# Snoworday/instance-segmentation-attention

Hardware: AMD Instinct MI355X
Metric: images/sec @256x256 bs=16 per GPU (higher is better)
Workload: dtype bf16; 1 GPU; train.py step fwd+bwd+update 256x256 bs=16/GPU (bf16); global_batch=16, parallelism=dp1, launch=hipGraph replay

## Files before the change

instance-segmentation-attention_amd/csrc/dwconv.hip:

```cpp
#include "common.hpp"
#include <type_traits>

namespace {

__device__ __forceinline__ void lds_barrier() {
    __builtin_amdgcn_fence(__ATOMIC_RELEASE, "workgroup", "local");
    __builtin_amdgcn_s_barrier();
    __builtin_amdgcn_fence(__ATOMIC_ACQUIRE, "workgroup", "local");
}

constexpr int TH = 8, TW = 32, CB = 32, PS = 36;
constexpr int HALO = (TH + 2) * (TW + 2);

struct Dw2Params {
    const void* x; const void* w; const float* bias; void* y; const void* dy;
    int n, h, w_, c, ldx, ldy, ldd, wld;
    ProDev pro;
    float* stats; int accumulate;
    int tiles_x, tiles_y; long ntiles;
    float* ws; int csrc;
    int G;
    FinDev fin;
};

// ... 18 lines not shown
    const int c0 = c_base + cg * 8;
    const bool cok = c0 < p.c;
    constexpr int NIT = (HALO * 4 + 255) / 256;
    float v[NIT][8];
    bool ok[NIT];
#pragma unroll
    for (int it = 0; it < NIT; ++it) {
        const int pix = (threadIdx.x + it * 256) >> 2;
        const int rr = pix / (TW + 2), cc = pix - rr * (TW + 2);
        const int gy = ty * TH + rr - 1, gx = tx * TW + cc - 1;
        ok[it] = pix < HALO && cok && gy >= 0 && gy < p.h && gx >= 0 && gx < p.w_;
        if (ok[it]) load8<T>(xin + (((long)b * p.h + gy) * p.w_ + gx) * p.ldx + c0, v[it]);
    }
#pragma unroll
    for (int it = 0; it < NIT; ++it) {
        const int pix = (threadIdx.x + it * 256) >> 2;
        if (pix >= HALO) continue;
        f32x4 a, bb;
#pragma unroll
        for (int j = 0; j < 8; ++j) {
            float z = 0.f;
            if (ok[it]) {
                z = v[it][j];
                if constexpr (HAS_PRO) {
                    z = act_t<ACT>(fmaf(z, r.sc[j], r.sh[j]), p.pro.act);
                    if (p.pro.bscale) z *= r.bs[j];
                }
            }
            if (j < 4) a[j] = z; else bb[j - 4] = z;
        }
        *reinterpret_cast<f32x4*>(tile + pix * PS + cg * 8) = a;
        *reinterpret_cast<f32x4*>(tile + pix * PS + cg * 8 + 4) = bb;
    }
}

typedef float f32x2 __attribute__((ext_vector_type(2)));
__device__ __forceinline__ void fma8(const float (&x)[8], const float (&w)[8], float (&acc)[8]) {
#ifdef ISA_DW_SCALAR_FMA
#pragma unroll
    for (int j = 0; j < 8; ++j) acc[j] = __builtin_fmaf(x[j], w[j], acc[j]);
#else
#pragma unroll
    for (int j = 0; j < 8; j += 2) {
        const f32x2 r = __builtin_elementwise_fma(f32x2{x[j], x[j + 1]}, f32x2{w[j], w[j + 1]}, f32x2{acc[j], acc[j + 1]});
        acc[j] = r[0]; acc[j + 1] = r[1];
    }
#endif
}

__device__ __forceinline__ void ld8(const float* p, float (&v)[8]) {
    const f32x4 a = *reinterpret_cast<const f32x4*>(p), b = *reinterpret_cast<const f32x4*>(p + 4);
#pragma unroll
    for (int j = 0; j < 4; ++j) { v[j] = a[j]; v[4 + j] = b[j]; }
}

struct TileRange { long t0, end, step; };
__device__ __forceinline__ TileRange tile_range(long ntiles, int bx, int nbx) {
    if ((nbx & 7) == 0 && ntiles >= 64) {
        const int xcd = bx & 7, j = bx >> 3;
        const long chunk = (ntiles + 7) / 8;
        const long end = min(ntiles, (xcd + 1) * chunk);
        return TileRange{xcd * chunk + j, end, (long)(nbx >> 3)};
    }
    return TileRange{(long)bx, ntiles, (long)nbx};
}

struct TileIter {
    long t, end, step;
    int tx, ty, b, sx, sy, sb, ntx, nty;
    __device__ __forceinline__ void init(const TileRange& r, int tiles_x, int tiles_y) {
        t = r.t0; end = r.end; step = r.step; ntx = tiles_x; nty = tiles_y;
        long q = t / tiles_x; tx = (int)(t - q * tiles_x); b = (int)(q / tiles_y); ty = (int)(q - (long)b * tiles_y);
        long qs = step / tiles_x; sx = (int)(step - qs * tiles_x); sb = (int)(qs / tiles_y); sy = (int)(qs - (long)sb * tiles_y);
    }
    __device__ __forceinline__ bool valid() const { return t < end; }
    __device__ __forceinline__ void next() {
        t += step;
        tx += sx; const int c = tx >= ntx ? 1 : 0; tx -= c * ntx;
        ty += sy + c; const int c2 = ty >= nty ? 1 : 0; ty -= c2 * nty;
        b += sb + c2;
    }
};

template <typename T, bool HAS_PRO, int ACT, bool DB>
__global__ __launch_bounds__(DB ? 768 : 256) __attribute__((amdgpu_waves_per_eu(2, 3))) void dw2_fwd_kernel(Dw2Params p) {
    constexpr int NTHR = DB ? 768 : 256;
    constexpr int LTHR = DB ? 512 : 256;
    constexpr int NBUF = DB ? 2 : 1;
    extern __shared__ __attribute__((aligned(16))) float sm[];
    float* tile_base = sm;
    float* wts = sm + NBUF * HALO * PS;
    float* red = wts + 9 * CB;
    float* fin_tab = red + 2 * CB;
    const int tid = threadIdx.x;
    const bool loader = DB && tid >= 256;
    const int ltid = loader ? tid - 256 : tid;
    const int c_base = blockIdx.y * CB;
    const GroupSel gs = group_sel(p.G);
    if (gs.g) {
        const long img = (long)gs.g * p.n, pix = img * p.h * p.w_;
        p.x = reinterpret_cast<const T*>(p.x) + pix * p.ldx;
        p.y = reinterpret_cast<T*>(p.y) + pix * p.ldy;
        p.pro.scale = goff(p.pro.scale, (long)gs.g * p.c); p.pro.shift = goff(p.pro.shift, (long)gs.g * p.c);
        p.pro.bscale = goff(p.pro.bscale, img * p.c);
        p.stats = goff(p.stats, (long)gs.g * ISA_STAT_R * 2 * p.c);
    }
    const T* wp = reinterpret_cast<const T*>(p.w);
    for (int i = tid; i < 9 * CB; i += NTHR) {
        const int tp = i / CB, cc = i - tp * CB;
        wts[i] = (c_base + cc < p.c) ? st<T>::ld(wp + (long)tp * p.wld + c_base + cc) : 0.f;
    }
    if (tid < 2 * CB) red[tid] = 0.f;
    const int cg = ltid & 3, g = ltid >> 2, row = g >> 3, x0 = (g & 7) * 4;
    const int c0 = c_base + cg * 8;
    const bool cok = c0 < p.c;
    const T* xin = reinterpret_cast<const T*>(p.x);
    constexpr int NIT = (HALO * 4 + LTHR - 1) / LTHR;

    const bool fin = HAS_PRO && bn_fin_inline<NTHR>(p.fin, p.c, p.G, gs.g, fin_tab, CB, tid, c_base, CB,
                                                    blockIdx.x == gridDim.x - 1 && blockIdx.z == 0);
    float sc[8], sh[8];
#pragma unroll
    for (int j = 0; j < 8; ++j) {
        const int c = min(c0 + j, p.c - 1);
        sc[j] = fin ? fin_tab[c - c_base] : ((HAS_PRO && p.pro.scale) ? p.pro.scale[c] : 1.f);
        sh[j] = fin ? fin_tab[CB + c - c_base] : ((HAS_PRO && p.pro.shift) ? p.pro.shift[c] : 0.f);
    }
    int hrc[NIT], hoff[NIT];
    bool hok[NIT];
#pragma unroll
    for (int it = 0; it < NIT; ++it) {
        const int pix = (ltid + it * LTHR) >> 2;
        const int rr = pix / (TW + 2), cc = pix - rr * (TW + 2);
        hrc[it] = (rr << 16) | cc;
        hoff[it] = (rr * p.w_ + cc) * p.ldx + (cok ? c0 : c_base);
        hok[it] = pix < HALO && cok;
    }
    const int ooff = (row * p.w_ + x0) * p.ldy + c0;

    auto stage = [&](int b, int ty, int tx, float* tile) {
        float bs[8];
        if (HAS_PRO && p.pro.bscale) {
#pragma unroll
            for (int j = 0; j < 8; ++j) bs[j] = p.pro.bscale[(long)b * p.c + min(c0 + j, p.c - 1)];
        }
        const T* base = xin + (((long)b * p.h + ty * TH - 1) * p.w_ + tx * TW - 1) * p.ldx;
        const int rlo = 1 - ty * TH, rhi = p.h + 1 - ty * TH, clo = 1 - tx * TW, chi = p.w_ + 1 - tx * TW;
        const bool interior = rlo <= 0 && rhi >= TH + 2 && clo <= 0 && chi >= TW + 2;
        raw8<T> v[NIT]; bool ok[NIT];
        if (interior) {
#pragma unroll
            for (int it = 0; it < NIT; ++it) { ok[it] = hok[it]; if (ok[it]) v[it].load(base + hoff[it]); }
        } else {
#pragma unroll
            for (int it = 0; it < NIT; ++it) {
                const int rr = hrc[it] >> 16, cc = hrc[it] & 0xffff;
                ok[it] = hok[it] && rr >= rlo && rr < rhi && cc >= clo && cc < chi;
                if (ok[it]) v[it].load(base + hoff[it]);
            }
        }
        const bool has_bs = HAS_PRO && p.pro.bscale;
#pragma unroll
        for (int it = 0; it < NIT; ++it) {
            const int pix = (ltid + it * LTHR) >> 2;
            if (pix >= HALO) continue;
            float o[8];
#pragma unroll
            for (int j = 0; j < 8; ++j) o[j] = 0.f;
            if (ok[it]) {
#pragma unroll
                for (int j = 0; j < 8; ++j) {
                    float z = v[it].get(j);
                    if constexpr (HAS_PRO) z = act_t<ACT>(fmaf(z, sc[j], sh[j]), p.pro.act);
                    o[j] = z;
                }
                if (has_bs) {
#pragma unroll
                    for (int j = 0; j < 8; ++j) o[j] *= bs[j];
                }
            }
            store8<float>(tile + pix * PS + cg * 8, o);
        }
    };

    auto compute = [&](int b, int ty, int tx, const float* tile, float (&s1)[8], float (&s2)[8]) {
        T* ybase = reinterpret_cast<T*>(p.y) + (((long)b * p.h + ty * TH) * p.w_ + tx * TW) * p.ldy;
        const bool rowok = ty * TH + row < p.h && cok;
        const int xlim = p.w_ - tx * TW;
        raw8<T> oc[4];
        if (p.accumulate && rowok) {
#pragma unroll
            for (int o = 0; o < 4; ++o)
                if (x0 + o < xlim) oc[o].load(ybase + ooff + o * p.ldy);
        }
        float acc[4][8];
        if (p.bias) {
#pragma unroll
            for (int o = 0; o < 4; ++o)
#pragma unroll
                for (int j = 0; j < 8; ++j) acc[o][j] = (c0 + j < p.c) ? p.bias[c0 + j] : 0.f;
        } else {
#pragma unroll
            for (int o = 0; o < 4; ++o)
#pragma unroll
                for (int j = 0; j < 8; ++j) acc[o][j] = 0.f;
        }
#pragma unroll 1
        for (int dy = 0; dy < 3; ++dy) {
            float wr[3][8], in[6][8];
#pragma unroll
            for (int k = 0; k < 3; ++k) ld8(wts + (dy * 3 + k) * CB + cg * 8, wr[k]);
#pragma unroll
            for (int k = 0; k < 6; ++k) ld8(tile + ((row + dy) * (TW + 2) + x0 + k) * PS + cg * 8, in[k]);
#pragma unroll
            for (int o = 0; o < 4; ++o)
#pragma unroll
                for (int k = 0; k < 3; ++k)
                    fma8(in[o + k], wr[k], acc[o]);
        }
        if (rowok) {
#pragma unroll
            for (int o = 0; o < 4; ++o) {
                if (x0 + o >= xlim) continue;
                T* dst = ybase + ooff + o * p.ldy;
#pragma unroll
                for (int j = 0; j < 8; ++j) { s1[j] += acc[o][j]; s2[j] += acc[o][j] * acc[o][j]; }
                if (p.accumulate) {
#pragma unroll
                    for (int j = 0; j < 8; ++j) acc[o][j] += oc[o].get(j);
                }
                store8<T>(dst, acc[o]);
            }
        }
    };

    __syncthreads();
    if (loader) {
        TileIter ti; ti.init(tile_range(p.ntiles, gs.bx, gs.nbx), p.tiles_x, p.tiles_y);
        int buf = 0;
        if (ti.valid()) stage(ti.b, ti.ty, ti.tx, tile_base);
        __syncthreads();
        while (ti.valid()) {
            ti.next();
            if (ti.valid()) stage(ti.b, ti.ty, ti.tx, tile_base + (buf ^ 1) * HALO * PS);
            lds_barrier();
            buf ^= 1;
        }
    } else {
        float s1[8] = {0, 0, 0, 0, 0, 0, 0, 0}, s2[8] = {0, 0, 0, 0, 0, 0, 0, 0};
        if constexpr (DB) {
            TileIter ti; ti.init(tile_range(p.ntiles, gs.bx, gs.nbx), p.tiles_x, p.tiles_y);
            int buf = 0;
            __syncthreads();
            for (; ti.valid(); ti.next()) {
                compute(ti.b, ti.ty, ti.tx, tile_base + buf * HALO * PS, s1, s2);
                lds_barrier();
                buf ^= 1;
            }
        } else {
            TileIter ti; ti.init(TileRange{(long)gs.bx, p.ntiles, (long)gs.nbx}, p.tiles_x, p.tiles_y);
            for (; ti.valid(); ti.next()) {
                stage(ti.b, ti.ty, ti.tx, tile_base);
                __syncthreads();
                compute(ti.b, ti.ty, ti.tx, tile_base, s1, s2);
                __syncthreads();
            }
        }
        if (p.stats) {
#pragma unroll
            for (int j = 0; j < 8; ++j) {
                s1[j] = row_fold<4>(s1[j]); s2[j] = row_fold<4>(s2[j]);
            }
            if ((tid & 15) < 4) {
#pragma unroll
                for (int j = 0; j < 8; ++j) { atomicAdd(&red[cg * 8 + j], s1[j]); atomicAdd(&red[CB + cg * 8 + j], s2[j]); }
            }
        }
    }
    __syncthreads();
    if (p.stats && tid < 2 * CB) {
        const int cc = tid & (CB - 1), which = tid / CB;
        if (c_base + cc < p.c && red[tid] != 0.f) {
            float* rep = p.stats + ((blockIdx.x + blockIdx.y) & (ISA_STAT_R - 1)) * 2 * p.c;
            atomicAdd(rep + which * p.c + c_base + cc, red[tid]);
        }
    }
}

template <typename T, bool HAS_PRO, int ACT>
__global__ __launch_bounds__(256) __attribute__((amdgpu_waves_per_eu(2, 2))) void dw2_wgrad_kernel(Dw2Params p) {
    extern __shared__ __attribute__((aligned(16))) float sm[];
    float* tile = sm;
    float* red = sm + HALO * PS;
    const int tid = threadIdx.x;
    const int c_base = blockIdx.y * CB;
    const int cg = tid & 3, g = tid >> 2, row = g >> 3, x0 = (g & 7) * 4;
    const int c0 = c_base + cg * 8;
    const GroupSel gs = group_sel(p.G);
    if (gs.g) {
        const long img = (long)gs.g * p.n, pix = img * p.h * p.w_;
        p.x = reinterpret_cast<const T*>(p.x) + pix * p.ldx;
        p.dy = reinterpret_cast<const T*>(p.dy) + pix * p.ldd;
        p.pro.scale = goff(p.pro.scale, (long)gs.g * p.c); p.pro.shift = goff(p.pro.shift, (long)gs.g * p.c);
        p.pro.bscale = goff(p.pro.bscale, img * p.c);
    }
    const T* din = reinterpret_cast<const T*>(p.dy);
    float acc[9][8], db[8];
#pragma unroll
    for (int tp = 0; tp < 9; ++tp)
#pragma unroll
        for (int j = 0; j < 8; ++j) acc[tp][j] = 0.f;
#pragma unroll
    for (int j = 0; j < 8; ++j) db[j] = 0.f;
    for (long t = gs.bx; t < p.ntiles; t += gs.nbx) {
        const int tx = (int)(t % p.tiles_x); const long q = t / p.tiles_x;
        const int ty = (int)(q % p.tiles_y); const int b = (int)(q / p.tiles_y);
        ProRegs pr;
        load_pro<HAS_PRO>(p, pr, c0, b);
        __syncthreads();
        stage_tile<T, HAS_PRO, ACT>(p, pr, tile, b, ty, tx, c_base);
        float d[4][8];
        const int oy = ty * TH + row;
#pragma unroll
        for (int o = 0; o < 4; ++o) {
            const int ox = tx * TW + x0 + o;
#pragma unroll
            for (int j = 0; j < 8; ++j) d[o][j] = 0.f;
            if (oy < p.h && ox < p.w_ && c0 < p.c) load8<T>(din + (((long)b * p.h + oy) * p.w_ + ox) * p.ldd + c0, d[o]);
        }
        __syncthreads();
#pragma unroll
        for (int o = 0; o < 4; ++o)
#pragma unroll
            for (int j = 0; j < 8; ++j) db[j] += d[o][j];
#pragma unroll
        for (int dy = 0; dy < 3; ++dy) {
            float in[6][8];
#pragma unroll
            for (int k = 0; k < 6; ++k) ld8(tile + ((row + dy) * (TW + 2) + x0 + k) * PS + cg * 8, in[k]);
#pragma unroll
            for (int o = 0; o < 4; ++o)
#pragma unroll
                for (int k = 0; k < 3; ++k)
                    fma8(in[o + k], d[o], acc[dy * 3 + k]);
            __builtin_amdgcn_sched_barrier(0);
        }
    }
    __syncthreads();
    for (int i = tid; i < 10 * CB; i += 256) red[i] = 0.f;
    __syncthreads();
#pragma unroll
    for (int tp = 0; tp < 10; ++tp) {
#pragma unroll
        for (int j = 0; j < 8; ++j) {
            float v = tp < 9 ? acc[tp < 9 ? tp : 0][j] : db[j];
            v = row_fold<4>(v);
            if ((tid & 15) < 4) atomicAdd(&red[tp * CB + cg * 8 + j], v);
        }
    }
    __syncthreads();
    float* slab = p.ws + ((long)blockIdx.x * gridDim.y + blockIdx.y) * 10 * CB;
    for (int i = tid; i < 10 * CB; i += 256) slab[i] = red[i];
}

constexpr int DW2_RSPLIT = 16;
__global__ __launch_bounds__(256) void dw2_wgrad_reduce_kernel(const float* ws, int nblk, int ncb, int C, int csrc, float* dw, float* dbias) {
    const int cb = blockIdx.x, split = blockIdx.y;
    const int per = (nblk + DW2_RSPLIT - 1) / DW2_RSPLIT;
    const int b0 = split * per, b1 = min(nblk, b0 + per);
    if (b0 >= b1) return;
    for (int i = threadIdx.x; i < 10 * CB; i += 256) {
        float s = 0.f;
#pragma unroll 8
        for (int b = b0; b < b1; ++b) s += ws[((long)b * ncb + cb) * 10 * CB + i];
        const int tp = i / CB, c = cb * CB + (i - tp * CB);
        if (c >= csrc || c >= C) continue;
        if (tp < 9) atomicAdd(dw + c * 9 + tp, s);
        else if (dbias) atomicAdd(dbias + c, s);
    }
}

template <typename T, bool HAS_PRO, int ACT>
int launch_fwd2_inst(Dw2Params& p, dim3 grid, hipStream_t s) {
    constexpr bool DB = sizeof(T) == 2;
    constexpr size_t lds = ((size_t)(DB ? 2 : 1) * HALO * PS + 9 * CB + 2 * CB + 2 * CB) * 4;
    static bool configured = false;
    if (!configured) {
        if (hipFuncSetAttribute(reinterpret_cast<const void*>(&dw2_fwd_kernel<T, HAS_PRO, ACT, DB>),
                                hipFuncAttributeMaxDynamicSharedMemorySize, (int)lds) != hipSuccess) return ISA_ELAUNCH;
        configured = true;
    }
    hipLaunchKernelGGL((dw2_fwd_kernel<T, HAS_PRO, ACT, DB>), grid, dim3(DB ? 768 : 256), lds, s, p);
    return launch_status();
}

template <typename T>
int launch_fwd2(Dw2Params& p, bool has_pro, hipStream_t s) {
    p.tiles_x = (p.w_ + TW - 1) / TW; p.tiles_y = (p.h + TH - 1) / TH;
    p.ntiles = (long)p.n * p.tiles_x * p.tiles_y;
    if (p.ntiles * p.G >= (1L << 31)) return ISA_EINVAL;
    const int ncb = (p.c + CB - 1) / CB;
    long gx = (256L * (sizeof(T) == 2 ? 1 : 3)) / ncb;
    if (gx < 1) gx = 1;
    if (gx > p.ntiles * p.G) gx = p.ntiles * p.G;
    gx = group_grid(gx, p.G);
    dim3 grid((unsigned)gx, ncb);
    if (has_pro && p.pro.act == ISA_ACT_RELU6) return launch_fwd2_inst<T, true, ISA_ACT_RELU6>(p, grid, s);
    if (has_pro) return launch_fwd2_inst<T, true, ACT_RT>(p, grid, s);
    return launch_fwd2_inst<T, false, ISA_ACT_NONE>(p, grid, s);
}

template <typename T>
int launch_wg2(Dw2Params& p, bool has_pro, long ws_floats, isa_slab_arena* sa, const isa_pro* fin, hipStream_t s) {
    p.tiles_x = (p.w_ + TW - 1) / TW; p.tiles_y = (p.h + TH - 1) / TH;
    p.ntiles = (long)p.n * p.tiles_x * p.tiles_y;
    const int ncb = (p.c + CB - 1) / CB;
    long gx = (256L * 2) / ncb;
    if (gx < 1) gx = 1;
    if (gx > p.ntiles * p.G) gx = p.ntiles * p.G;
    if (int rc = defer_ws(sa, &p.ws, &ws_floats)) return rc;
    const long ws_cap = ws_floats / (10L * CB * ncb);
    if (ws_cap < p.G) return sa ? ISA_ENOMEM : ISA_EINVAL;
    if (gx > ws_cap) gx = ws_cap;
    gx = group_grid(gx, p.G);
    dim3 grid((unsigned)gx, ncb);
    const size_t lds = ((size_t)HALO * PS + 10 * CB) * 4;
    if (int rc = fin_standalone(fin, p.c, p.G, s)) return rc;
    if (has_pro && p.pro.act == ISA_ACT_RELU6) hipLaunchKernelGGL((dw2_wgrad_kernel<T, true, ISA_ACT_RELU6>), grid, dim3(256), lds, s, p);
    else if (has_pro) hipLaunchKernelGGL((dw2_wgrad_kernel<T, true, ACT_RT>), grid, dim3(256), lds, s, p);
    else hipLaunchKernelGGL((dw2_wgrad_kernel<T, false, ISA_ACT_NONE>), grid, dim3(256), lds, s, p);
    if (launch_status() != ISA_OK) return ISA_ELAUNCH;
    if (defer_push(sa, FoldDesc{p.ws, (float*)p.y, (float*)p.bias, nullptr, 1, (int)gx, ncb, 9, 1, 0, CB, p.c, 0, p.csrc, 0, 0, 0, 0},
                   gx * ncb * 10L * CB)) return ISA_OK;
    hipLaunchKernelGGL(dw2_wgrad_reduce_kernel, dim3(ncb, DW2_RSPLIT), dim3(256), 0, s, p.ws, (int)gx, ncb, p.c, p.csrc, (float*)p.y, (float*)p.bias);
    return launch_status();
}


struct FusedParams {
    const void *g, *y, *x, *w; void* dx;
    int n, h, w_, c, ldg, ldy, ldx, lddx, wld;
    const float *ysc, *ysh, *ymu, *yis, *yred; float ycnt_inv; int yact; float *ydgamma, *ydbeta;
    const float *xsc, *xsh, *xmu, *xis; int xact; float* xred;
    int accumulate, tiles_x, tiles_y; long ntiles; float* ws; int csrc; float* dw;
    const void* addend; int lda;
    int G;
};


template <typename T> struct dd_stride { static constexpr int v = 36; };
template <> struct dd_stride<bf16_t> { static constexpr int v = 40; };

template <typename T, int YACT, int XMODE, bool DB, bool EPI>
__global__ __launch_bounds__(DB ? 512 : 256) __attribute__((amdgpu_waves_per_eu(2, 2))) void dw_bn_bwd_kernel(FusedParams p) {
    constexpr int PSD = dd_stride<T>::v;
    constexpr int XACT = XMODE == 1 ? ISA_ACT_RELU6 : (XMODE == 0 ? ISA_ACT_NONE : ACT_RT);
    constexpr int NBUF = DB ? 2 : 1;
    constexpr int NTHR = DB ? 512 : 256;
    constexpr int TILE_ELEMS = HALO * PSD;
    extern __shared__ __attribute__((aligned(16))) float sm[];
    T* xt_base = reinterpret_cast<T*>(sm);
    T* dt_base = xt_base + NBUF * TILE_ELEMS;
    float* wts = reinterpret_cast<float*>(dt_base + NBUF * TILE_ELEMS);
    float* cst = wts + 9 * CB;
    float* red = cst + 10 * CB;
    const int tid = threadIdx.x;
    const int ltid = tid & 255;
    const bool loader = DB && tid >= 256;
    const int c_base = blockIdx.y * CB;
    const GroupSel gs = group_sel(p.G);
    if (gs.g) {
        const long pix = (long)gs.g * p.n * p.h * p.w_, gc = (long)gs.g * p.c;
        p.g = reinterpret_cast<const T*>(p.g) + pix * p.ldg; p.y = reinterpret_cast<const T*>(p.y) + pix * p.ldy;
        p.x = reinterpret_cast<const T*>(p.x) + pix * p.ldx; p.dx = reinterpret_cast<T*>(p.dx) + pix * p.lddx;
        if (p.addend) p.addend = reinterpret_cast<const T*>(p.addend) + pix * p.lda;
        p.ysc += gc; p.ysh += gc; p.ymu += gc; p.yis += gc; p.yred += gc * ISA_STAT_R * 2;
        p.xsc = goff(p.xsc, gc); p.xsh = goff(p.xsh, gc); p.xmu = goff(p.xmu, gc); p.xis = goff(p.xis, gc);
        p.xred = goff(p.xred, gc * ISA_STAT_R * 2);
    }
    const int cg = ltid & 3, g4 = ltid >> 2, row = g4 >> 3, x0 = (g4 & 7) * 4;
    const int c0 = c_base + cg * 8;
    const bool cok = c0 < p.c;
    const T* wp = reinterpret_cast<const T*>(p.w);
    for (int i = tid; i < 9 * CB; i += NTHR) {
        const int tp = i / CB, cc = i - tp * CB;
        wts[i] = (c_base + cc < p.c) ? st<T>::ld(wp + (long)tp * p.wld + c_base + cc) : 0.f;
    }
    if (tid < CB) {
        const int c = min(c_base + tid, p.c - 1);
        cst[0 * CB + tid] = p.ysc[c]; cst[1 * CB + tid] = p.ysh[c];
        cst[2 * CB + tid] = p.ymu[c]; cst[3 * CB + tid] = p.yis[c];
        float r0 = 0.f, r1 = 0.f;
#pragma unroll
        for (int r = 0; r < ISA_STAT_R; ++r) { r0 += p.yred[r * 2 * p.c + c]; r1 += p.yred[r * 2 * p.c + p.c + c]; }
        cst[4 * CB + tid] = r0 * p.ycnt_inv; cst[5 * CB + tid] = r1 * p.ycnt_inv;
        cst[6 * CB + tid] = (XMODE && p.xsc) ? p.xsc[c] : 1.f; cst[7 * CB + tid] = (XMODE && p.xsh) ? p.xsh[c] : 0.f;
        cst[8 * CB + tid] = (XMODE && p.xmu) ? p.xmu[c] : 0.f; cst[9 * CB + tid] = (XMODE && p.xis) ? p.xis[c] : 1.f;
        if (gs.bx == 0 && c_base + tid < p.c) {
            if (p.ydgamma) atomicAdd(p.ydgamma + c, r1);
            if (p.ydbeta) atomicAdd(p.ydbeta + c, r0);
        }
    }
    for (int i = tid; i < 11 * CB; i += NTHR) red[i] = 0.f;
    const T* gin = reinterpret_cast<const T*>(p.g);
    const T* yin = reinterpret_cast<const T*>(p.y);
    const T* xin = reinterpret_cast<const T*>(p.x);
    T* dxo = reinterpret_cast<T*>(p.dx);
    constexpr int NIT = (HALO * 4 + 255) / 256;
    constexpr int NB = 3;
    static_assert(NIT % NB == 0, "staging chunks");
    const bool want_xred = XMODE == 1 || (XMODE == 2 && p.xred != nullptr);

    int hrc[NIT], hog[NIT], hoy[NIT], hox[NIT];
    bool hok[NIT];
#pragma unroll
    for (int it = 0; it < NIT; ++it) {
        const int pix = (ltid + it * 256) >> 2;
        const int rr = pix / (TW + 2), cc = pix - rr * (TW + 2);
        const int cc0 = cok ? c0 : c_base;
        hrc[it] = (rr << 16) | cc;
        hog[it] = (rr * p.w_ + cc) * p.ldg + cc0;
        hoy[it] = (rr * p.w_ + cc) * p.ldy + cc0;
        hox[it] = (rr * p.w_ + cc) * p.ldx + cc0;
        hok[it] = pix < HALO && cok;
    }
    const int oodx = (row * p.w_ + x0) * p.lddx + c0, ooa = (row * p.w_ + x0) * p.lda + c0;

    struct Geo { const T *gb, *yb, *xb; int rlo, rhi, clo, chi, sg, sy, sx; bool interior; };
    auto geo = [&](int b, int ty, int tx) {
        Geo g;
        const long horg = ((long)b * p.h + ty * TH - 1) * p.w_ + tx * TW - 1;
        g.gb = gin + horg * p.ldg; g.yb = yin + horg * p.ldy; g.xb = xin + horg * p.ldx;
        g.rlo = 1 - ty * TH; g.rhi = p.h + 1 - ty * TH; g.clo = 1 - tx * TW; g.chi = p.w_ + 1 - tx * TW;
        g.interior = g.rlo <= 0 && g.rhi >= TH + 2 && g.clo <= 0 && g.chi >= TW + 2;
        const int cc0 = cok ? c0 : c_base;
        g.sg = (p.w_ + 1) * p.ldg + cc0; g.sy = (p.w_ + 1) * p.ldy + cc0; g.sx = (p.w_ + 1) * p.ldx + cc0;
        return g;
    };
    auto slot_ok = [&](const Geo& g, int it) {
        const int rr = hrc[it] >> 16, cc = hrc[it] & 0xffff;
        return hok[it] && (g.interior || (rr >= g.rlo && rr < g.rhi && cc >= g.clo && cc < g.chi));
    };
    struct StageK { float sc[8], sh[8], mu[8], is[8], k0[8], k1[8]; };
    auto convert = [&](bool ok, int it, const StageK& K, const raw8<T>& gv, const raw8<T>& yv, const raw8<T>& xv, T* xt, T* dt) {
        const int pix = (ltid + it * 256) >> 2;
        if (pix >= HALO) return;
        float o[8];
        raw8<T> q = xv;
#pragma unroll
        for (int j = 0; j < 8; ++j) {
            const float yy = yv.get(j);
            const float z = fmaf(yy, K.sc[j], K.sh[j]);
            const float dz = gv.get(j) * act_grad_t<YACT>(z, p.yact);
            const float yh = (yy - K.mu[j]) * K.is[j];
            o[j] = K.sc[j] * (dz - K.k0[j] - yh * K.k1[j]);
        }
        if (__builtin_amdgcn_ballot_w64(!ok) != 0) {
#pragma unroll
            for (int j = 0; j < 8; ++j) o[j] = ok ? o[j] : 0.f;
            if (!ok) q.zero();
        }
        store8<T>(dt + pix * PSD + cg * 8, o);
        q.store(xt + pix * PSD + cg * 8);
    };
    auto issue = [&](const Geo& g, int it, raw8<T>& gv, raw8<T>& yv, raw8<T>& xv) {
        const bool ok = slot_ok(g, it);
        gv.load(g.gb + (ok ? hog[it] : g.sg));
        yv.load(g.yb + (ok ? hoy[it] : g.sy));
        xv.load(g.xb + (ok ? hox[it] : g.sx));
        asm volatile("" ::: "memory");
    };

    auto stage = [&](int b, int ty, int tx, T* xt, T* dt) {
        const Geo g = geo(b, ty, tx);
        StageK K;
        ld8(cst + 0 * CB + cg * 8, K.sc); ld8(cst + 1 * CB + cg * 8, K.sh); ld8(cst + 2 * CB + cg * 8, K.mu);
        ld8(cst + 3 * CB + cg * 8, K.is); ld8(cst + 4 * CB + cg * 8, K.k0); ld8(cst + 5 * CB + cg * 8, K.k1);
#pragma unroll
        for (int it0 = 0; it0 < NIT; it0 += NB) {
            raw8<T> gv[NB], yv[NB], xv[NB];
#pragma unroll
            for (int u = 0; u < NB; ++u) issue(g, it0 + u, gv[u], yv[u], xv[u]);
#pragma unroll
            for (int u = 0; u < NB; ++u) convert(slot_ok(g, it0 + u), it0 + u, K, gv[u], yv[u], xv[u], xt, dt);
            __builtin_amdgcn_sched_barrier(0);
        }
    };

    auto compute = [&](int b, int ty, int tx, const T* xt, const T* dt, float (&acc)[9][8], float (&s0)[8], float (&s1)[8]) {
        const long torg = ((long)b * p.h + ty * TH) * p.w_ + tx * TW;
        T* dxb = dxo + torg * p.lddx + oodx;
        const T* adb = reinterpret_cast<const T*>(p.addend) + torg * p.lda + ooa;
        const bool rowok = ty * TH + row < p.h && cok;
        const int xlim = p.w_ - tx * TW;
        raw8<T> oc[4], ad[4];
        if constexpr (EPI) {
            if (rowok) {
#pragma unroll
                for (int o = 0; o < 4; ++o) {
                    if (x0 + o >= xlim) continue;
                    if (p.accumulate) oc[o].load(dxb + o * p.lddx);
                    if constexpr (XMODE == 0) { if (p.addend) ad[o].load(adb + o * p.lda); }
                }
            }
        }
        {
            float a[4][8];
#pragma unroll
            for (int o = 0; o < 4; ++o)
#pragma unroll
                for (int j = 0; j < 8; ++j) a[o][j] = 0.f;
#pragma unroll 1
            for (int dy = 0; dy < 3; ++dy) {
                float wr[3][8], in[6][8];
#pragma unroll
                for (int k = 0; k < 3; ++k) ld8(wts + (dy * 3 + k) * CB + cg * 8, wr[k]);
#pragma unroll
                for (int k = 0; k < 6; ++k) load8<T>(dt + ((row + dy) * (TW + 2) + x0 + k) * PSD + cg * 8, in[k]);
#pragma unroll
                for (int o = 0; o < 4; ++o)
#pragma unroll
                    for (int k = 0; k < 3; ++k)
                        fma8(in[o + k], wr[k], a[o]);
            }
            if (rowok) {
                float xs[8], xh[8], xm[8], xi[8];
                if (want_xred) {
                    ld8(cst + 6 * CB + cg * 8, xs); ld8(cst + 7 * CB + cg * 8, xh);
                    ld8(cst + 8 * CB + cg * 8, xm); ld8(cst + 9 * CB + cg * 8, xi);
                }
#pragma unroll
                for (int o = 0; o < 4; ++o) {
                    if (x0 + o >= xlim) continue;
                    T* dst = dxb + o * p.lddx;
                    if constexpr (EPI) {
                        if (p.accumulate) {
#pragma unroll
                            for (int j = 0; j < 8; ++j) a[o][j] += oc[o].get(j);
                        }
                        if constexpr (XMODE == 0) {
                            if (p.addend) {
#pragma unroll
                                for (int j = 0; j < 8; ++j) a[o][j] += ad[o].get(j);
                            }
                        }
                    }
                    store8<T>(dst, a[o]);
                    if (want_xred) {
                        float xr[8];
                        load8<T>(xt + ((row + 1) * (TW + 2) + x0 + 1 + o) * PSD + cg * 8, xr);
#pragma unroll
                        for (int j = 0; j < 8; ++j) {
                            const float gq = (float)(T)a[o][j];
                            const float z = fmaf(xr[j], xs[j], xh[j]);
                            const float dz = gq * act_grad_t<XACT>(z, p.xact);
                            s0[j] += dz; s1[j] += dz * ((xr[j] - xm[j]) * xi[j]);
                        }
                    }
                }
            }
        }
        __builtin_amdgcn_sched_barrier(0);
        {
            float d[4][8];
#pragma unroll
            for (int o = 0; o < 4; ++o) load8<T>(dt + ((row + 1) * (TW + 2) + x0 + 1 + o) * PSD + cg * 8, d[o]);
            float ps[8], ph[8];
            if constexpr (XMODE != 0) { ld8(cst + 6 * CB + cg * 8, ps); ld8(cst + 7 * CB + cg * 8, ph); }
            const int rlo = 1 - ty * TH, rhi = p.h + 1 - ty * TH, clo = 1 - tx * TW, chi = p.w_ + 1 - tx * TW;
            const bool interior = XMODE == 0 || (rlo <= 0 && rhi >= TH + 2 && clo <= 0 && chi >= TW + 2);
            auto window = [&](auto border) {
                constexpr bool BORDER = decltype(border)::value;
#pragma unroll
                for (int dy = 0; dy < 3; ++dy) {
                    const bool row_in = row + dy >= rlo && row + dy < rhi;
#pragma unroll
                    for (int k = 0; k < 6; ++k) {
                        float in[8];
                        load8<T>(xt + ((row + dy) * (TW + 2) + x0 + k) * PSD + cg * 8, in);
                        if constexpr (XMODE != 0) {
                            float z[8];
#pragma unroll
                            for (int j = 0; j < 8; ++j) z[j] = ph[j];
                            fma8(in, ps, z);
#pragma unroll
                            for (int j = 0; j < 8; ++j) in[j] = act_t<XACT>(z[j], p.xact);
                            if constexpr (BORDER) {
                                const bool in_img = row_in && x0 + k >= clo && x0 + k < chi;
#pragma unroll
                                for (int j = 0; j < 8; ++j) in[j] = in_img ? in[j] : 0.f;
                            }
                        }
#pragma unroll
                        for (int o = 0; o < 4; ++o)
                            if (k - o >= 0 && k - o < 3) fma8(in, d[o], acc[dy * 3 + (k - o)]);
                    }
                    __builtin_amdgcn_sched_barrier(0);
                }
            };
            if (interior) window(std::false_type{});
            else window(std::true_type{});
        }
    };

    __syncthreads();
    if (loader) {
        StageK K;
        ld8(cst + 0 * CB + cg * 8, K.sc); ld8(cst + 1 * CB + cg * 8, K.sh); ld8(cst + 2 * CB + cg * 8, K.mu);
        ld8(cst + 3 * CB + cg * 8, K.is); ld8(cst + 4 * CB + cg * 8, K.k0); ld8(cst + 5 * CB + cg * 8, K.k1);
        TileIter tn; tn.init(tile_range(p.ntiles, gs.bx, gs.nbx), p.tiles_x, p.tiles_y);
        raw8<T> gv[NIT], yv[NIT], xv[NIT];
        Geo gs, gn;
        bool have = tn.valid();
        if (have) {
            gn = geo(tn.b, tn.ty, tn.tx);
#pragma unroll
            for (int it = 0; it < NIT; ++it) issue(gn, it, gv[it], yv[it], xv[it]);
        }
        int buf = 0;
        while (have) {
            gs = gn;
            tn.next();
            T* xt = xt_base + buf * TILE_ELEMS; T* dt = dt_base + buf * TILE_ELEMS;
            if (tn.valid()) {
                gn = geo(tn.b, tn.ty, tn.tx);
#pragma unroll
                for (int it = 0; it < NIT; ++it) {
                    convert(slot_ok(gs, it), it, K, gv[it], yv[it], xv[it], xt, dt);
                    issue(gn, it, gv[it], yv[it], xv[it]);
                }
            } else {
#pragma unroll
                for (int it = 0; it < NIT; ++it) convert(slot_ok(gs, it), it, K, gv[it], yv[it], xv[it], xt, dt);
                have = false;
            }
            lds_barrier();
            buf ^= 1;
        }
        lds_barrier();
    } else {
        float acc[9][8], s0[8], s1[8];
#pragma unroll
        for (int tp = 0; tp < 9; ++tp)
#pragma unroll
            for (int j = 0; j < 8; ++j) acc[tp][j] = 0.f;
#pragma unroll
        for (int j = 0; j < 8; ++j) { s0[j] = 0.f; s1[j] = 0.f; }
        if constexpr (DB) {
            TileIter ti; ti.init(tile_range(p.ntiles, gs.bx, gs.nbx), p.tiles_x, p.tiles_y);
            int buf = 0;
            lds_barrier();
            for (; ti.valid(); ti.next()) {
                compute(ti.b, ti.ty, ti.tx, xt_base + buf * TILE_ELEMS, dt_base + buf * TILE_ELEMS, acc, s0, s1);
                lds_barrier();
                buf ^= 1;
            }
        } else {
            TileIter ti; ti.init(TileRange{(long)gs.bx, p.ntiles, (long)gs.nbx}, p.tiles_x, p.tiles_y);
            for (; ti.valid(); ti.next()) {
                stage(ti.b, ti.ty, ti.tx, xt_base, dt_base);
                __syncthreads();
                compute(ti.b, ti.ty, ti.tx, xt_base, dt_base, acc, s0, s1);
                __syncthreads();
            }
        }
        float* part = reinterpret_cast<float*>(sm);
        const int slot = cg * 16 + (tid >> 6) * 4 + ((tid >> 4) & 3);
        const bool writer = (tid & 15) < 4;
#pragma unroll
        for (int tp = 0; tp < 9; ++tp) {
#pragma unroll
            for (int j = 0; j < 8; ++j) {
                const float v = row_fold<4>(acc[tp][j]);
                if (writer) part[(tp * 8 + j) * 64 + slot] = v;
            }
        }
#pragma unroll
        for (int j = 0; j < 8; ++j) {
            const float v0 = row_fold<4>(s0[j]), v1 = row_fold<4>(s1[j]);
            if (writer) { part[(72 + j) * 64 + slot] = v0; part[(80 + j) * 64 + slot] = v1; }
        }
    }
    __syncthreads();
    {
        const float* part = reinterpret_cast<const float*>(sm);
        for (int o = tid; o < 88 * 4; o += NTHR) {
            const f32x4 a = *reinterpret_cast<const f32x4*>(part + o * 16), b = *reinterpret_cast<const f32x4*>(part + o * 16 + 4),
                        c = *reinterpret_cast<const f32x4*>(part + o * 16 + 8), d = *reinterpret_cast<const f32x4*>(part + o * 16 + 12);
            const f32x4 t = (a + b) + (c + d);
            const int v = o >> 2, g = o & 3;
            red[(v >> 3) * CB + g * 8 + (v & 7)] = (t[0] + t[1]) + (t[2] + t[3]);
        }
    }
    __syncthreads();
    float* slab = p.ws + ((long)blockIdx.x * gridDim.y + blockIdx.y) * 10 * CB;
    for (int i = tid; i < 10 * CB; i += NTHR) slab[i] = i < 9 * CB ? red[i] : 0.f;
    if (want_xred && tid < 2 * CB) {
        const int cc = tid & (CB - 1), which = tid / CB;
        const float v = red[9 * CB + tid];
        if (c_base + cc < p.c && v != 0.f) {
            float* rep = p.xred + ((blockIdx.x + blockIdx.y) & (ISA_STAT_R - 1)) * 2 * p.c;
// ... 149 lines not shown
```

Baseline: 717.1 images/s.

## Prefetch dwconv halo tiles ahead of prologue and split accumulate path into template

The forward depthwise conv loader warps now issue global loads for the first tile(s) before the prologue (weights, bias, BN scale/shift, fin) and keep a register prefetch pipeline that converts one tile while loading the next. Loads are made unconditional by pointing out-of-bounds slots at a safe address, and zeros are applied afterwards. Per-image bscale is cached and prefetched, and bias is hoisted into registers. Accumulate becomes a compile-time template flag. The backward kernel similarly issues its first tile loads before constant/weight setup. Extra registers and more complex control flow may hurt occupancy.

```diff
diff --git a/instance-segmentation-attention_amd/csrc/dwconv.hip b/instance-segmentation-attention_amd/csrc/dwconv.hip
--- a/instance-segmentation-attention_amd/csrc/dwconv.hip
+++ b/instance-segmentation-attention_amd/csrc/dwconv.hip
@@ -124,11 +124,17 @@
     }
 };
 
-template <typename T, bool HAS_PRO, int ACT, bool DB>
+#ifndef ISA_DW_FWD_PF
+#define ISA_DW_FWD_PF 1
+#endif
+
+template <typename T, bool HAS_PRO, int ACT, bool DB, bool ACC>
 __global__ __launch_bounds__(DB ? 768 : 256) __attribute__((amdgpu_waves_per_eu(2, 3))) void dw2_fwd_kernel(Dw2Params p) {
     constexpr int NTHR = DB ? 768 : 256;
     constexpr int LTHR = DB ? 512 : 256;
     constexpr int NBUF = DB ? 2 : 1;
+    constexpr int PF = ISA_DW_FWD_PF;
+    static_assert(PF == 1 || PF == 2, "prefetch distance in tiles");
     extern __shared__ __attribute__((aligned(16))) float sm[];
     float* tile_base = sm;
     float* wts = sm + NBUF * HALO * PS;
@@ -136,6 +142,7 @@
     float* fin_tab = red + 2 * CB;
     const int tid = threadIdx.x;
     const bool loader = DB && tid >= 256;
+    const bool stager = !DB || loader;
     const int ltid = loader ? tid - 256 : tid;
     const int c_base = blockIdx.y * CB;
     const GroupSel gs = group_sel(p.G);
@@ -148,26 +155,14 @@
         p.stats = goff(p.stats, (long)gs.g * ISA_STAT_R * 2 * p.c);
     }
     const T* wp = reinterpret_cast<const T*>(p.w);
-    for (int i = tid; i < 9 * CB; i += NTHR) {
-        const int tp = i / CB, cc = i - tp * CB;
-        wts[i] = (c_base + cc < p.c) ? st<T>::ld(wp + (long)tp * p.wld + c_base + cc) : 0.f;
-    }
-    if (tid < 2 * CB) red[tid] = 0.f;
     const int cg = ltid & 3, g = ltid >> 2, row = g >> 3, x0 = (g & 7) * 4;
     const int c0 = c_base + cg * 8;
     const bool cok = c0 < p.c;
+    const int cc0 = cok ? c0 : c_base;
     const T* xin = reinterpret_cast<const T*>(p.x);
     constexpr int NIT = (HALO * 4 + LTHR - 1) / LTHR;
-
-    const bool fin = HAS_PRO && bn_fin_inline<NTHR>(p.fin, p.c, p.G, gs.g, fin_tab, CB, tid, c_base, CB,
-                                                    blockIdx.x == gridDim.x - 1 && blockIdx.z == 0);
-    float sc[8], sh[8];
-#pragma unroll
-    for (int j = 0; j < 8; ++j) {
-        const int c = min(c0 + j, p.c - 1);
-        sc[j] = fin ? fin_tab[c - c_base] : ((HAS_PRO && p.pro.scale) ? p.pro.scale[c] : 1.f);
-        sh[j] = fin ? fin_tab[CB + c - c_base] : ((HAS_PRO && p.pro.shift) ? p.pro.shift[c] : 0.f);
-    }
+    const bool has_bs = HAS_PRO && p.pro.bscale;
+
     int hrc[NIT], hoff[NIT];
     bool hok[NIT];
 #pragma unroll
@@ -175,54 +170,115 @@
         const int pix = (ltid + it * LTHR) >> 2;
         const int rr = pix / (TW + 2), cc = pix - rr * (TW + 2);
         hrc[it] = (rr << 16) | cc;
-        hoff[it] = (rr * p.w_ + cc) * p.ldx + (cok ? c0 : c_base);
+        hoff[it] = (rr * p.w_ + cc) * p.ldx + cc0;
         hok[it] = pix < HALO && cok;
     }
+    const int soff = (p.w_ + 1) * p.ldx + cc0;
     const int ooff = (row * p.w_ + x0) * p.ldy + c0;
 
+    struct Geo { const T* base; int b, rlo, rhi, clo, chi; bool interior; };
+    auto geo = [&](int b, int ty, int tx) {
+        Geo q;
+        q.base = xin + (((long)b * p.h + ty * TH - 1) * p.w_ + tx * TW - 1) * p.ldx;
+        q.b = b;
+        q.rlo = 1 - ty * TH; q.rhi = p.h + 1 - ty * TH; q.clo = 1 - tx * TW; q.chi = p.w_ + 1 - tx * TW;
+        q.interior = q.rlo <= 0 && q.rhi >= TH + 2 && q.clo <= 0 && q.chi >= TW + 2;
+        return q;
+    };
+    auto slot_ok = [&](const Geo& q, int it) {
+        const int rr = hrc[it] >> 16, cc = hrc[it] & 0xffff;
+        return hok[it] && (q.interior || (rr >= q.rlo && rr < q.rhi && cc >= q.clo && cc < q.chi));
+    };
+    auto issue = [&](const Geo& q, int it, raw8<T>& v) {
+        v.load(q.base + (slot_ok(q, it) ? hoff[it] : soff));
+        asm volatile("" ::: "memory");
+    };
+
+    float bv[8], sc[8], sh[8], bs[8];
+    auto prologue = [&](int b_first) {
+    const float* dummy = reinterpret_cast<const float*>(p.x);
+    constexpr int NW = (9 * CB + NTHR - 1) / NTHR;
+    float wv[NW];
+#pragma unroll
+    for (int k = 0; k < NW; ++k) {
+        const int i = min(tid + k * NTHR, 9 * CB - 1);
+        const int tp = i / CB, cc = i - tp * CB;
+        wv[k] = st<T>::ld(wp + (long)tp * p.wld + min(c_base + cc, p.c - 1));
+    }
+    const bool fin_pending = HAS_PRO && p.fin.stats != nullptr;
+    const bool ld_sc = HAS_PRO && p.pro.scale && !fin_pending, ld_sh = HAS_PRO && p.pro.shift && !fin_pending;
+    if (!loader) {
+        const float* bp = p.bias ? p.bias : dummy;
+#pragma unroll
+        for (int j = 0; j < 8; ++j) bv[j] = bp[p.bias ? min(c0 + j, p.c - 1) : 0];
+    }
+    if (HAS_PRO && stager) {
+        const float* sp = ld_sc ? p.pro.scale : dummy;
+        const float* hp = ld_sh ? p.pro.shift : dummy;
+        const float* mp = (DB && has_bs) ? p.pro.bscale + (long)b_first * p.c : dummy;
+#pragma unroll
+        for (int j = 0; j < 8; ++j) {
+            const int c = min(c0 + j, p.c - 1);
+            sc[j] = sp[ld_sc ? c : 0];
+            sh[j] = hp[ld_sh ? c : 0];
+            if constexpr (DB) bs[j] = mp[has_bs ? c : 0];
+        }
+    }
+    asm volatile("" ::: "memory");
+    const bool fin = HAS_PRO && bn_fin_inline<NTHR>(p.fin, p.c, p.G, gs.g, fin_tab, CB, tid, c_base, CB,
+                                                    blockIdx.x == gridDim.x - 1 && blockIdx.z == 0);
+#pragma unroll
+    for (int k = 0; k < NW; ++k) {
+        const int i = tid + k * NTHR;
+        if (i < 9 * CB) wts[i] = (c_base + (i & (CB - 1)) < p.c) ? wv[k] : 0.f;
+    }
+    if (tid < 2 * CB) red[tid] = 0.f;
+#pragma unroll
+    for (int j = 0; j < 8; ++j) {
+        const int c = min(c0 + j, p.c - 1);
+        bv[j] = (p.bias && c0 + j < p.c) ? bv[j] : 0.f;
+        sc[j] = ld_sc ? sc[j] : 1.f;
+        sh[j] = ld_sh ? sh[j] : 0.f;
+        if (fin) { sc[j] = fin_tab[c - c_base]; sh[j] = fin_tab[CB + c - c_base]; }
+        bs[j] = (DB && has_bs) ? bs[j] : 1.f;
+    }
+    __syncthreads();
+    };
+
+    auto convert = [&](bool ok, int it, const raw8<T>& r, float* tile) {
+        const int pix = (ltid + it * LTHR) >> 2;
+        if (pix >= HALO) return;
+        float o[8];
+#pragma unroll
+        for (int j = 0; j < 8; ++j) {
+            float z = r.get(j);
+            if constexpr (HAS_PRO) z = act_t<ACT>(fmaf(z, sc[j], sh[j]), p.pro.act);
+            o[j] = z;
+        }
+        if constexpr (HAS_PRO) {
+#pragma unroll
+            for (int j = 0; j < 8; ++j) o[j] *= bs[j];
+        }
+        if (__builtin_amdgcn_ballot_w64(!ok) != 0) {
+#pragma unroll
+            for (int j = 0; j < 8; ++j) o[j] = ok ? o[j] : 0.f;
+        }
+        store8<float>(tile + pix * PS + cg * 8, o);
+    };
+
+    int bs_img = -1;
     auto stage = [&](int b, int ty, int tx, float* tile) {
-        float bs[8];
-        if (HAS_PRO && p.pro.bscale) {
+        if (has_bs && b != bs_img) {
 #pragma unroll
             for (int j = 0; j < 8; ++j) bs[j] = p.pro.bscale[(long)b * p.c + min(c0 + j, p.c - 1)];
-        }
-        const T* base = xin + (((long)b * p.h + ty * TH - 1) * p.w_ + tx * TW - 1) * p.ldx;
-        const int rlo = 1 - ty * TH, rhi = p.h + 1 - ty * TH, clo = 1 - tx * TW, chi = p.w_ + 1 - tx * TW;
-        const bool interior = rlo <= 0 && rhi >= TH + 2 && clo <= 0 && chi >= TW + 2;
-        raw8<T> v[NIT]; bool ok[NIT];
-        if (interior) {
-#pragma unroll
-            for (int it = 0; it < NIT; ++it) { ok[it] = hok[it]; if (ok[it]) v[it].load(base + hoff[it]); }
-        } else {
-#pragma unroll
-            for (int it = 0; it < NIT; ++it) {
-                const int rr = hrc[it] >> 16, cc = hrc[it] & 0xffff;
-                ok[it] = hok[it] && rr >= rlo && rr < rhi && cc >= clo && cc < chi;
-                if (ok[it]) v[it].load(base + hoff[it]);
-            }
-        }
-        const bool has_bs = HAS_PRO && p.pro.bscale;
-#pragma unroll
-        for (int it = 0; it < NIT; ++it) {
-            const int pix = (ltid + it * LTHR) >> 2;
-            if (pix >= HALO) continue;
-            float o[8];
-#pragma unroll
-            for (int j = 0; j < 8; ++j) o[j] = 0.f;
-            if (ok[it]) {
-#pragma unroll
-                for (int j = 0; j < 8; ++j) {
-                    float z = v[it].get(j);
-                    if constexpr (HAS_PRO) z = act_t<ACT>(fmaf(z, sc[j], sh[j]), p.pro.act);
-                    o[j] = z;
-                }
-                if (has_bs) {
-#pragma unroll
-                    for (int j = 0; j < 8; ++j) o[j] *= bs[j];
-                }
-            }
-            store8<float>(tile + pix * PS + cg * 8, o);
-        }
+            bs_img = b;
+        }
+        const Geo q = geo(b, ty, tx);
+        raw8<T> r[NIT];
+#pragma unroll
+        for (int it = 0; it < NIT; ++it) issue(q, it, r[it]);
+#pragma unroll
+        for (int it = 0; it < NIT; ++it) convert(slot_ok(q, it), it, r[it], tile);
     };
 
     auto compute = [&](int b, int ty, int tx, const float* tile, float (&s1)[8], float (&s2)[8]) {
@@ -230,23 +286,16 @@
         const bool rowok = ty * TH + row < p.h && cok;
         const int xlim = p.w_ - tx * TW;
         raw8<T> oc[4];
-        if (p.accumulate && rowok) {
-#pragma unroll
-            for (int o = 0; o < 4; ++o)
-                if (x0 + o < xlim) oc[o].load(ybase + ooff + o * p.ldy);
+        if constexpr (ACC) {
+#pragma unroll
+            for (int o = 0; o < 4; ++o) oc[o].load(ybase + ((rowok && x0 + o < xlim) ? ooff + o * p.ldy : cc0));
+            asm volatile("" ::: "memory");
         }
         float acc[4][8];
-        if (p.bias) {
-#pragma unroll
-            for (int o = 0; o < 4; ++o)
-#pragma unroll
-                for (int j = 0; j < 8; ++j) acc[o][j] = (c0 + j < p.c) ? p.bias[c0 + j] : 0.f;
-        } else {
-#pragma unroll
-            for (int o = 0; o < 4; ++o)
-#pragma unroll
-                for (int j = 0; j < 8; ++j) acc[o][j] = 0.f;
-        }
+#pragma unroll
+        for (int o = 0; o < 4; ++o)
+#pragma unroll
+            for (int j = 0; j < 8; ++j) acc[o][j] = bv[j];
 #pragma unroll 1
         for (int dy = 0; dy < 3; ++dy) {
             float wr[3][8], in[6][8];
@@ -267,7 +316,7 @@
                 T* dst = ybase + ooff + o * p.ldy;
 #pragma unroll
                 for (int j = 0; j < 8; ++j) { s1[j] += acc[o][j]; s2[j] += acc[o][j] * acc[o][j]; }
-                if (p.accumulate) {
+                if constexpr (ACC) {
 #pragma unroll
                     for (int j = 0; j < 8; ++j) acc[o][j] += oc[o].get(j);
                 }
@@ -276,24 +325,84 @@
         }
     };
 
-    __syncthreads();
     if (loader) {
-        TileIter ti; ti.init(tile_range(p.ntiles, gs.bx, gs.nbx), p.tiles_x, p.tiles_y);
-        int buf = 0;
-        if (ti.valid()) stage(ti.b, ti.ty, ti.tx, tile_base);
-        __syncthreads();
-        while (ti.valid()) {
-            ti.next();
-            if (ti.valid()) stage(ti.b, ti.ty, ti.tx, tile_base + (buf ^ 1) * HALO * PS);
+        if constexpr (DB) {
+            TileIter tn;
+            Geo gq[PF];
+            bool val[PF];
+            raw8<T> v[PF][NIT];
+            tn.init(tile_range(p.ntiles, gs.bx, gs.nbx), p.tiles_x, p.tiles_y);
+#pragma unroll
+            for (int d = 0; d < PF; ++d) {
+                val[d] = tn.valid();
+                gq[d] = val[d] ? geo(tn.b, tn.ty, tn.tx) : geo(0, 0, 0);
+#pragma unroll
+                for (int it = 0; it < NIT; ++it) issue(gq[d], it, v[d][it]);
+                tn.next();
+            }
+            prologue(gq[0].b);
+            float bsn[8];
+            bool bs_new = false;
+            TileIter tb;
+            if (has_bs) { tb.init(tile_range(p.ntiles, gs.bx, gs.nbx), p.tiles_x, p.tiles_y); tb.next(); }
+            int buf = 0;
+            auto step = [&](auto dsel, auto refill) {
+                constexpr int d = decltype(dsel)::value;
+                constexpr bool REFILL = decltype(refill)::value;
+                float* tile = tile_base + buf * HALO * PS;
+                const Geo gc = gq[d];
+                if (has_bs) {
+                    if (bs_new) {
+#pragma unroll
+                        for (int j = 0; j < 8; ++j) bs[j] = bsn[j];
+                    }
+                    bs_new = tb.valid() && tb.b != gc.b;
+                    if (bs_new) {
+#pragma unroll
+                        for (int j = 0; j < 8; ++j) bsn[j] = p.pro.bscale[(long)tb.b * p.c + min(c0 + j, p.c - 1)];
+                        asm volatile("" ::: "memory");
+                    }
+                    tb.next();
+                }
+                if constexpr (REFILL) {
+                    gq[d] = geo(tn.b, tn.ty, tn.tx);
+#pragma unroll
+                    for (int it = 0; it < NIT; ++it) {
+                        convert(slot_ok(gc, it), it, v[d][it], tile);
+                        issue(gq[d], it, v[d][it]);
+                    }
+                    tn.next();
+                } else {
+#pragma unroll
+                    for (int it = 0; it < NIT; ++it) convert(slot_ok(gc, it), it, v[d][it], tile);
+                    val[d] = false;
+                }
+                lds_barrier();
+                buf ^= 1;
+            };
+            while (tn.t + (PF - 1) * tn.step < tn.end) {
+                step(std::integral_constant<int, 0>{}, std::true_type{});
+                if constexpr (PF > 1) step(std::integral_constant<int, 1>{}, std::true_type{});
+            }
+            while (val[0]) {
+                if (PF > 1 && tn.valid()) step(std::integral_constant<int, 0>{}, std::true_type{});
+                else step(std::integral_constant<int, 0>{}, std::false_type{});
+                if constexpr (PF > 1) {
+                    if (val[1]) {
+                        if (tn.valid()) step(std::integral_constant<int, 1>{}, std::true_type{});
+                        else step(std::integral_constant<int, 1>{}, std::false_type{});
+                    }
+                }
+            }
             lds_barrier();
-            buf ^= 1;
         }
     } else {
+        prologue(0);
         float s1[8] = {0, 0, 0, 0, 0, 0, 0, 0}, s2[8] = {0, 0, 0, 0, 0, 0, 0, 0};
         if constexpr (DB) {
             TileIter ti; ti.init(tile_range(p.ntiles, gs.bx, gs.nbx), p.tiles_x, p.tiles_y);
             int buf = 0;
-            __syncthreads();
+            lds_barrier();
             for (; ti.valid(); ti.next()) {
                 compute(ti.b, ti.ty, ti.tx, tile_base + buf * HALO * PS, s1, s2);
                 lds_barrier();
@@ -422,17 +531,17 @@
     }
 }
 
-template <typename T, bool HAS_PRO, int ACT>
+template <typename T, bool HAS_PRO, int ACT, bool ACC = false>
 int launch_fwd2_inst(Dw2Params& p, dim3 grid, hipStream_t s) {
     constexpr bool DB = sizeof(T) == 2;
     constexpr size_t lds = ((size_t)(DB ? 2 : 1) * HALO * PS + 9 * CB + 2 * CB + 2 * CB) * 4;
     static bool configured = false;
     if (!configured) {
-        if (hipFuncSetAttribute(reinterpret_cast<const void*>(&dw2_fwd_kernel<T, HAS_PRO, ACT, DB>),
+        if (hipFuncSetAttribute(reinterpret_cast<const void*>(&dw2_fwd_kernel<T, HAS_PRO, ACT, DB, ACC>),
                                 hipFuncAttributeMaxDynamicSharedMemorySize, (int)lds) != hipSuccess) return ISA_ELAUNCH;
         configured = true;
     }
-    hipLaunchKernelGGL((dw2_fwd_kernel<T, HAS_PRO, ACT, DB>), grid, dim3(DB ? 768 : 256), lds, s, p);
+    hipLaunchKernelGGL((dw2_fwd_kernel<T, HAS_PRO, ACT, DB, ACC>), grid, dim3(DB ? 768 : 256), lds, s, p);
     return launch_status();
 }
 
@@ -447,6 +556,7 @@
     if (gx > p.ntiles * p.G) gx = p.ntiles * p.G;
     gx = group_grid(gx, p.G);
     dim3 grid((unsigned)gx, ncb);
+    if (p.accumulate) return has_pro ? ISA_EINVAL : launch_fwd2_inst<T, false, ISA_ACT_NONE, true>(p, grid, s);
     if (has_pro && p.pro.act == ISA_ACT_RELU6) return launch_fwd2_inst<T, true, ISA_ACT_RELU6>(p, grid, s);
     if (has_pro) return launch_fwd2_inst<T, true, ACT_RT>(p, grid, s);
     return launch_fwd2_inst<T, false, ISA_ACT_NONE>(p, grid, s);
@@ -524,26 +634,6 @@
     const int c0 = c_base + cg * 8;
     const bool cok = c0 < p.c;
     const T* wp = reinterpret_cast<const T*>(p.w);
-    for (int i = tid; i < 9 * CB; i += NTHR) {
-        const int tp = i / CB, cc = i - tp * CB;
-        wts[i] = (c_base + cc < p.c) ? st<T>::ld(wp + (long)tp * p.wld + c_base + cc) : 0.f;
-    }
-    if (tid < CB) {
-        const int c = min(c_base + tid, p.c - 1);
-        cst[0 * CB + tid] = p.ysc[c]; cst[1 * CB + tid] = p.ysh[c];
-        cst[2 * CB + tid] = p.ymu[c]; cst[3 * CB + tid] = p.yis[c];
-        float r0 = 0.f, r1 = 0.f;
-#pragma unroll
-        for (int r = 0; r < ISA_STAT_R; ++r) { r0 += p.yred[r * 2 * p.c + c]; r1 += p.yred[r * 2 * p.c + p.c + c]; }
-        cst[4 * CB + tid] = r0 * p.ycnt_inv; cst[5 * CB + tid] = r1 * p.ycnt_inv;
-        cst[6 * CB + tid] = (XMODE && p.xsc) ? p.xsc[c] : 1.f; cst[7 * CB + tid] = (XMODE && p.xsh) ? p.xsh[c] : 0.f;
-        cst[8 * CB + tid] = (XMODE && p.xmu) ? p.xmu[c] : 0.f; cst[9 * CB + tid] = (XMODE && p.xis) ? p.xis[c] : 1.f;
-        if (gs.bx == 0 && c_base + tid < p.c) {
-            if (p.ydgamma) atomicAdd(p.ydgamma + c, r1);
-            if (p.ydbeta) atomicAdd(p.ydbeta + c, r0);
-        }
-    }
-    for (int i = tid; i < 11 * CB; i += NTHR) red[i] = 0.f;
     const T* gin = reinterpret_cast<const T*>(p.g);
     const T* yin = reinterpret_cast<const T*>(p.y);
     const T* xin = reinterpret_cast<const T*>(p.x);
@@ -613,6 +703,59 @@
         asm volatile("" ::: "memory");
     };
 
+    TileIter tn;
+    raw8<T> gv[NIT], yv[NIT], xv[NIT];
+    Geo gn;
+    if constexpr (DB) {
+        if (loader) {
+            tn.init(tile_range(p.ntiles, gs.bx, gs.nbx), p.tiles_x, p.tiles_y);
+            if (tn.valid()) {
+                gn = geo(tn.b, tn.ty, tn.tx);
+#pragma unroll
+                for (int it = 0; it < NIT; ++it) issue(gn, it, gv[it], yv[it], xv[it]);
+            }
+        }
+    }
+    constexpr int NW = (9 * CB + NTHR - 1) / NTHR;
+    float wv[NW];
+#pragma unroll
+    for (int k = 0; k < NW; ++k) {
+        const int i = min(tid + k * NTHR, 9 * CB - 1);
+        const int tp = i / CB, cc = i - tp * CB;
+        wv[k] = st<T>::ld(wp + (long)tp * p.wld + min(c_base + cc, p.c - 1));
+    }
+    if (tid < CB) {
+        const int c = min(c_base + tid, p.c - 1);
+        const bool hsc = XMODE && p.xsc, hsh = XMODE && p.xsh, hmu = XMODE && p.xmu, his = XMODE && p.xis;
+        const float ysc = p.ysc[c], ysh = p.ysh[c], ymu = p.ymu[c], yis = p.yis[c];
+        float ra[ISA_STAT_R], rb[ISA_STAT_R];
+#pragma unroll
+        for (int r = 0; r < ISA_STAT_R; ++r) { ra[r] = p.yred[r * 2 * p.c + c]; rb[r] = p.yred[r * 2 * p.c + p.c + c]; }
+        float xsc = 1.f, xsh = 0.f, xmu = 0.f, xis = 1.f;
+        if constexpr (XMODE != 0) {
+            xsc = (hsc ? p.xsc : p.ysc)[c]; xsh = (hsh ? p.xsh : p.ysc)[c];
+            xmu = (hmu ? p.xmu : p.ysc)[c]; xis = (his ? p.xis : p.ysc)[c];
+        }
+        asm volatile("" ::: "memory");
+        cst[0 * CB + tid] = ysc; cst[1 * CB + tid] = ysh; cst[2 * CB + tid] = ymu; cst[3 * CB + tid] = yis;
+        float r0 = 0.f, r1 = 0.f;
+#pragma unroll
+        for (int r = 0; r < ISA_STAT_R; ++r) { r0 += ra[r]; r1 += rb[r]; }
+        cst[4 * CB + tid] = r0 * p.ycnt_inv; cst[5 * CB + tid] = r1 * p.ycnt_inv;
+        cst[6 * CB + tid] = hsc ? xsc : 1.f; cst[7 * CB + tid] = hsh ? xsh : 0.f;
+        cst[8 * CB + tid] = hmu ? xmu : 0.f; cst[9 * CB + tid] = his ? xis : 1.f;
+        if (gs.bx == 0 && c_base + tid < p.c) {
+            if (p.ydgamma) atomicAdd(p.ydgamma + c, r1);
+            if (p.ydbeta) atomicAdd(p.ydbeta + c, r0);
+        }
+    }
+#pragma unroll
+    for (int k = 0; k < NW; ++k) {
+        const int i = tid + k * NTHR;
+        if (i < 9 * CB) wts[i] = (c_base + (i & (CB - 1)) < p.c) ? wv[k] : 0.f;
+    }
+    for (int i = tid; i < 11 * CB; i += NTHR) red[i] = 0.f;
+
     auto stage = [&](int b, int ty, int tx, T* xt, T* dt) {
         const Geo g = geo(b, ty, tx);
         StageK K;
@@ -750,15 +893,8 @@
         StageK K;
         ld8(cst + 0 * CB + cg * 8, K.sc); ld8(cst + 1 * CB + cg * 8, K.sh); ld8(cst + 2 * CB + cg * 8, K.mu);
         ld8(cst + 3 * CB + cg * 8, K.is); ld8(cst + 4 * CB + cg * 8, K.k0); ld8(cst + 5 * CB + cg * 8, K.k1);
-        TileIter tn; tn.init(tile_range(p.ntiles, gs.bx, gs.nbx), p.tiles_x, p.tiles_y);
-        raw8<T> gv[NIT], yv[NIT], xv[NIT];
-        Geo gs, gn;
+        Geo gs;
         bool have = tn.valid();
-        if (have) {
-            gn = geo(tn.b, tn.ty, tn.tx);
-#pragma unroll
-            for (int it = 0; it < NIT; ++it) issue(gn, it, gv[it], yv[it], xv[it]);
-        }
         int buf = 0;
         while (have) {
             gs = gn;
```

Measured after the change: 726.1 images/s, median of 6. 1.3% higher.
